# albertz/ParseOggVorbis

Measured on AMD Instinct MI355X. Metric: audio packets/sec (blocksize 2048, stereo), higher is better.
Workload: dtype f32; 1 GPU; config3: 65536 stereo packets, blocksize 2048, 64 streams x 1024, floor+coupling+IMDCT+window+overlap-add; packets_per_gpu=65536, parallelism=streams sharded over 1 GPU(s), no data-path collective

## Files before the change

parseoggvorbis_amd/csrc/vorbis_synth_hip.hip:

```cpp
#include <hip/hip_runtime.h>

#include <math.h>
#include <stdarg.h>
#include <stdio.h>
#include <string.h>

#include <algorithm>
#include <cmath>
#include <mutex>
#include <numeric>
#include <string>
#include <vector>

#include <stdlib.h>

#include "vsyn_device.h"
#include "vsyn_staged.h"
#include "vsyn_prep.h"
#include "vsyn_fused.h"
#include "vsyn_fused_u.h"
#include "vsyn_vq.h"
#include "vsyn_pcm.h"
#include "vsyn_features.h"
#include "vsyn_spectral.h"
// ... 486 lines not shown
        for (int i = 0; i + 1 < VQ_NSTAMPS; ++i) sum[i] += (double)host[u][i];
      }
      if (pk) {
        fprintf(stderr, "[vq stamps] %llu waves, %.1f packets each; s_memtime ticks per packet:", waves, (double)pk / waves);
        for (int i = 0; i + 1 < VQ_NSTAMPS; ++i) fprintf(stderr, " %d:%.0f", i, sum[i] / pk);
        fprintf(stderr, "\n");
      }
    }
  }
#endif
#ifdef PREP_STAMPS
  {
    static unsigned long long host[8192][PREP_NSTAMPS];
    if (hipMemcpyFromSymbol(host, HIP_SYMBOL(g_prep_stamps), sizeof(host)) == hipSuccess) {
      unsigned long long t_first = ~0ull;
      for (int u = 0; u < 8192; ++u)
        if (host[u][7] && host[u][5] < t_first) t_first = host[u][5];
      for (unsigned role = 0; role < 2; ++role) {
        double sum[5] = {0}, st = 0, en = 0, en_max = 0, st_max = 0;
        unsigned long long waves = 0;
        for (int u = 0; u < 8192; ++u) {
          if (host[u][7] != 1ull + role) continue;
          ++waves;
          for (int i = 0; i < 5; ++i) sum[i] += (double)host[u][i];
          const double a = (double)(host[u][5] - t_first) / 100.0, b = (double)(host[u][6] - t_first) / 100.0;
          st += a;
          en += b;
          if (a > st_max) st_max = a;
          if (b > en_max) en_max = b;
        }
        if (!waves) continue;
        static const char* nm[5] = {"header + stream state", "scan in front of the chunk", "descriptors, scan, PktInfo", "floor role: descriptors, floor ids", "floor role: chains"};
        fprintf(stderr, "prep stamps, %s role: %llu waves; start %.2f us (latest %.2f), end %.2f us (latest %.2f) after the launch's first wave\n",
                role ? "floor" : "layout", waves, st / waves, st_max, en / waves, en_max);
        for (int i = 0; i < 5; ++i)
          if (sum[i] > 0) fprintf(stderr, "  %-36s %8.0f cycles\n", nm[i], sum[i] / waves);
      }
    }
  }
#endif
#ifdef VSYN_STAMPS
  {
    static unsigned long long host[8192][VSYN_NSTAMPS];
    if (hipMemcpyFromSymbol(host, HIP_SYMBOL(g_vsyn_stamps), sizeof(host)) == hipSuccess) {
      double sum[VSYN_NSTAMPS] = {0};
      unsigned long long waves = 0, pk = 0;
      for (int u = 0; u < 8192; ++u) {
        if (!host[u][VSYN_NSTAMPS - 1]) continue;
        ++waves;
        pk += host[u][VSYN_NSTAMPS - 1];
        for (int i = 0; i + 1 < VSYN_NSTAMPS; ++i) sum[i] += (double)host[u][i];
      }
      if (pk) {
        static const char* nm[VSYN_NSTAMPS - 1] = {"loop", "residue+handoff+couple", "loads+floor setup", "floor product", "mirror+pre-rot", "partner wait 2",
                                                   "fft512", "post+window+overlap", "stores / short pass: stores", "short: descriptors", "short: rows", "short: couple+floor", "short: fft+window", "-", "-"};
        double tot = 0;
        for (int i = 0; i + 1 < VSYN_NSTAMPS; ++i) tot += sum[i];
        fprintf(stderr, "vsyn stamps: %llu waves, %llu wave-packets, %.0f cycles per wave-packet\n", waves, pk, tot / pk);
        for (int i = 0; i + 1 < VSYN_NSTAMPS; ++i) fprintf(stderr, "  %-26s %8.0f cycles  %5.1f %%\n", nm[i], sum[i] / pk, 100.0 * sum[i] / tot);
      }
    }
  }
#endif
  fused_tables_destroy(&h->fused);
  u_tables_destroy(&h->utab);
  if (h->side) (void)hipStreamDestroy(h->side);
  if (h->pre) (void)hipStreamDestroy(h->pre);
  if (h->host_stream) (void)hipStreamDestroy(h->host_stream);
  if (h->ev_join) (void)hipEventDestroy(h->ev_join);
  if (h->ev_self) (void)hipEventDestroy(h->ev_self);
  if (h->ev_reset) (void)hipEventDestroy(h->ev_reset);
  for (uint32_t b = 0; b < vsyn_handle::WS_RING; ++b)
    if (h->ev_pre_done[b]) (void)hipEventDestroy(h->ev_pre_done[b]);
  for (uint32_t b = 0; b < vsyn_handle::EV_RING; ++b)
    if (h->ev_ring[b]) (void)hipEventDestroy(h->ev_ring[b]);
  if (h->d_const) (void)hipFree(h->d_const);
  if (h->d_vq) (void)hipFree(h->d_vq);
  h->st_curve.release(); h->st_vqpk.release(); h->st_cls.release(); h->st_ent.release();
  if (h->d_state) (void)hipFree(h->d_state);
  if (h->d_carry) (void)hipFree(h->d_carry);
  if (h->d_status) (void)hipFree(h->d_status);
  h->ws_count.release();
  h->ws_chunks.release();
  for (uint32_t b = 0; b < vsyn_handle::WS_RING; ++b) {
    h->ws_list[b].release(); h->ws_info[b].release(); h->ws_seg[b].release(); h->ws_segmap[b].release(); h->ws_fy[b].release(); h->ws_runcls[b].release();
  }
  h->ws_env.release(); h->ws_blk.release();
  h->st_pk.release(); h->st_seg.release(); h->st_ys.release(); h->st_fy.release(); h->st_res.release(); h->st_pcm.release();
  h->st_env.release(); h->st_blk.release(); h->st_emit.release();
  h->st_sum.release(); h->st_conv.release(); h->st_frames.release();
  for (auto& ev : h->events) {
    (void)hipEventDestroy(ev.first);
    (void)hipEventDestroy(ev.second);
  }
  delete h;
}

uint32_t vsyn_ys_stride(const vsyn_handle* h) { return h ? h->H.ys_stride : 0; }
uint32_t vsyn_channels(const vsyn_handle* h) { return h ? h->H.channels : 0; }
uint32_t vsyn_fused_paths(const vsyn_handle* h) { return h ? (h->fused_mask | (h->vq_tables_in_lds ? 0x100u : 0u)) : 0; }
size_t vsyn_const_block_bytes(const vsyn_handle* h) { return h ? h->host_const.size() : 0; }

int vsyn_profile_enable(vsyn_handle* h, int on) {
  if (!h) return VSYN_ERR_INVALID;
  h->profile = on != 0;
  if (on >= 1 && on <= 3) h->profile_which = on;
  return VSYN_OK;
}

int vsyn_profile_read(vsyn_handle* h, double* mean_ms, uint32_t* launches, const char** kernel_name) {
  if (!h) return VSYN_ERR_INVALID;
  std::lock_guard<std::mutex> lk(h->mu);
// ... 1695 lines not shown
```

parseoggvorbis_amd/csrc/vsyn_fused.h:

```cpp
#pragma once
#include <hip/hip_runtime.h>

#include "vsyn_device.h"

#ifndef FUSED_WAVES
#define FUSED_WAVES 16
#endif
#ifndef FUSED_MIN_WAVES_PER_SIMD
#define FUSED_MIN_WAVES_PER_SIMD 4
#endif
#define FUSED_XSLOTS 576
#ifndef VSYN_KNOCKOUT
#define VSYN_KNOCKOUT 0
#endif
#ifdef VSYN_STAMPS
#define VSYN_NSTAMPS 16
__device__ unsigned long long g_vsyn_stamps[8192][VSYN_NSTAMPS];
#define STAMP(i)                                                  \
  do {                                                            \
    __builtin_amdgcn_sched_barrier(0);                            \
    const unsigned long long t_ = __builtin_readcyclecounter();   \
    st_acc[i] += t_ - st_last;                                    \
    st_last = t_;                                                 \
    __builtin_amdgcn_sched_barrier(0);                            \
  } while (0)
#else
#define STAMP(i) do { } while (0)
#endif

struct FusedLdsImage {
  float2 pre[8][64];
  float2 post[8][64];
  float2 tw1[8][64];
  float2 tw2[8][8];
  float win[2][2][8][64];
  float invdb[260];
  float2 pre_s[64];
  float2 post_s[64];
  float2 tws[6][64];
  float wsl[2][64];
  float2 post8[8][8];
  float wsl8[2][8][8];
};

struct FusedTables {
  uint8_t* d_binseg = nullptr;
  FusedLdsImage* d_lds = nullptr;
  int waves_per_cu = 12;
  int coupling_mode = 0;
};

struct FusedArgs {
  const uint8_t* cb;
  const uint8_t* binseg;
  const FusedLdsImage* lds_image;
  const vsyn_packet* packets;
  const vsyn_segment* segs;
  const PktInfo* info;
  const SegInfo* sinfo;
  uint16_t* curve;
  const uint8_t* run_cls;
  const float* residue;
  const uint16_t* fy;
  float* pcm;
  float* carry;
  DevStatus* status;
  uint64_t plane_stride;
  uint32_t S, R, fused_ok, coupling_mode, runs_per_seg;
};
// ... 73 lines not shown
  asm volatile("" ::: "memory");
  uint32_t spins = 0;
  while (!dead && *(const volatile lds_u32*)flag < v) {
    __builtin_amdgcn_s_sleep(2);
    if (++spins > (1u << 24)) {
      if ((threadIdx.x & 63u) == 0) atomicOr(&status->flags, VSYN_ST_BAD_SEGMENT);
      dead = true;
    }
  }
  asm volatile("" ::: "memory");
}

__device__ __forceinline__ float min0(float a) {
  float r;
  asm("v_min_f32 %0, 0, %1" : "=v"(r) : "v"(a));
  return r;
}
__device__ __forceinline__ float max0(float a) {
  float r;
  asm("v_max_f32 %0, 0, %1" : "=v"(r) : "v"(a));
  return r;
}
__device__ __forceinline__ float couple_mag(float m, float a) {
  const float na = min0(a);
  return m + (m > 0.f ? na : -na);
}
__device__ __forceinline__ float couple_ang(float m, float a) {
  const float pa = max0(a);
  return m + (m > 0.f ? -pa : pa);
}

typedef uint32_t u32x8 __attribute__((ext_vector_type(8)));
static_assert(sizeof(PktInfo) == 32, "PktInfo is fetched as one s_load_dwordx8");
struct PktScalars {
  uint64_t res_off;
  uint32_t out_pos, emit, used, own, widx, mapping, lng, bad;
};
__device__ __forceinline__ PktScalars pkt_fields(const u32x8 r) {
  PktScalars k;
  k.res_off = (uint64_t)r[0] | ((uint64_t)r[1] << 32);
  k.out_pos = r[2];
  k.emit = r[3];
  k.used = r[4];
  k.own = r[5];
  k.widx = r[6] >> 24;
  k.mapping = r[7] & 0xFFu;
  k.lng = (r[6] >> 16) & 0xFFu;
  k.bad = (r[7] >> 8) & 0xFFu;
  return k;
}
__device__ __forceinline__ PktScalars pkt_load(const PktInfo* p) {
  typedef const __attribute__((address_space(4))) u32x8* const_words;
  return pkt_fields(*(const_words)(uintptr_t)p);
}

enum { K_REG = 0, K_LDS = 1, K_CARRY = 2 };
__device__ __forceinline__ uint32_t bitrev6(uint32_t l) { return __brev(l) >> 26; }

template <int ROLE, bool TAPC>
__device__ __forceinline__ uint32_t fused_short_pass(const FusedArgs& A, const FusedLdsImage& T, float2* __restrict__ xb, const float2* __restrict__ pxb,
                                                     float2* seg2, lds_f32* cbuf, lds_u32* my_flags, const lds_u32* partner_flags, const uint32_t lane,
                                                     const vsyn_segment sg, const SegInfo si, const uint32_t q, const uint32_t qa, const uint32_t qb,
                                                     const uint32_t C, const uint32_t c, float* plane, const PktInfo* ip, const uint32_t epoch,
                                                     const uint32_t prev_kind, const uint32_t prev_half, float (&P)[8], const uint32_t bseg0,
                                                     const uint32_t sidx, const uint32_t xsl, const uint32_t posts, const uint32_t ys_stride, bool& hand_over_out
#ifdef VSYN_STAMPS
                                                     , unsigned long long (&st_acc)[VSYN_NSTAMPS], unsigned long long& st_last
#endif
                                                     ) {
  constexpr uint32_t MS = 128u, ML = 1024u;
  const ConstHeader* H = hdr_of(A.cb);
  typedef uint32_t u32x4 __attribute__((ext_vector_type(4)));
  const uint32_t idx = min(q + (lane & 7u), qb - 1u);
  const u32x4 da = ((const u32x4*)(ip + idx))[0], db = ((const u32x4*)(ip + idx))[1];
  const uint32_t map0 = __builtin_amdgcn_readfirstlane(db[3] & 0xFFu);
  const bool cand = lane < 8u && q + lane < qb;
  const uint64_t okm = __ballot(cand && !((db[3] >> 8) & 0xFFu) && !((db[2] >> 16) & 0xFFu) && (db[3] & 0xFFu) == map0);
  const uint32_t Jp = (uint32_t)__builtin_ctzll(~okm);
  STAMP(9);
  const uint32_t qn = q + Jp, p0 = sg.first_packet + q;
  const uint32_t emit_l = q + (lane & 7u) < qa ? 0u : da[3];
  float2 raw[8];
  uint32_t vrow[8];
#pragma unroll
  for (uint32_t t = 0; t < 8; ++t) {
    const uint32_t tc = min(t, Jp - 1u);
    const uint64_t off = ((uint64_t)__builtin_amdgcn_readlane(da[1], tc) << 32) | (uint32_t)__builtin_amdgcn_readlane(da[0], tc);
    raw[t] = (VSYN_KNOCKOUT & 256) ? f2(0.001f * (float)lane, 0.002f) : ((const float2*)(A.residue + off + (size_t)c * MS))[lane];
    vrow[t] = (A.fy + ((size_t)(p0 + tc) * C + c) * ys_stride)[sidx];
  }
#pragma unroll
  for (uint32_t t = 0; t < 8; ++t)
    if (t >= Jp) raw[t] = f2(0.f, 0.f);
  float2 r[8];
  if (ROLE != 0 && !(VSYN_KNOCKOUT & 512)) {
#pragma unroll
    for (int t = 0; t < 8; ++t) xb[t * 64 + lane] = raw[t];
    STAMP(10);
    pair_post(&my_flags[0], epoch);
    pair_wait(&partner_flags[0], epoch);
#pragma unroll
    for (int t = 0; t < 8; ++t) {
      const float2 oth = pxb[t * 64 + lane];
      r[t] = ROLE == 1 ? f2(couple_mag(raw[t].x, oth.x), couple_mag(raw[t].y, oth.y)) : f2(couple_ang(oth.x, raw[t].x), couple_ang(oth.y, raw[t].y));
    }
    pair_post(&my_flags[1], epoch);
// ... 163 lines not shown
          *(float2*)(up + 16 * j) = f2(oh_s[j], n_s[j]);
          *(float2*)(dn - 16 * j) = f2(n_m[j], oh_m[j]);
        }
      }
    } else if (emit) {
#pragma unroll
      for (int j = 0; j < 4; ++j) {
        const uint32_t s = 2u * kap + 16u * j;
        const uint32_t f0 = s + shift, f1 = s + 1u + shift, f2m = MS - 2u - s + shift, f3m = MS - 1u - s + shift;
        if (f0 < emit) out[f0] = oh_s[j];
        if (f1 < emit) out[f1] = n_s[j];
        if (f2m < emit) out[f2m] = n_m[j];
        if (f3m < emit) out[f3m] = oh_m[j];
      }
    }
  }
  (void)next_emit;
  (void)next_out;
  if ((last_of_segment || hand_over) && jo == Jp - 1u) {
    const size_t carry_half = (size_t)H->max_streams * C * ML;
    float* cout = A.carry + (si.parity_in ^ 1u) * carry_half + ((size_t)sg.stream * C + c) * ML;
#pragma unroll
    for (int k = 0; k < 8; ++k) {
      const uint32_t f = kap + 8u * k;
      const uint32_t s = k >= 4 ? 2u * f - 64u : 63u - 2u * f, sm = MS - 1u - s;
      const float v_s = Pn[k] * wl1[k], v_m = Pn[k] * wl0[k];
      if (last_of_segment) {
        cout[s] = v_s;
        cout[sm] = v_m;
      } else {
        cbuf[s] = v_s;
        cbuf[sm] = v_m;
      }
    }
  }
  {
    const int from = (int)((Jp - 1u) * 8u + kap);
#pragma unroll
    for (int k = 0; k < 8; ++k) P[k] = __shfl(Pn[k], from);
  }
  if (__any(floor_bad)) {
    if (floor_bad) raise_status(A.status, VSYN_ST_FLOOR_VALUE, floor_bad_pkt);
    vmem_drain();
  }
  hand_over_out = hand_over;
  return Jp;
}


template <int ROLE, bool MIXED, bool TAPC, bool RING = false>
__device__ __forceinline__ void fused_run(const FusedArgs& A, const FusedLdsImage& T, float2* __restrict__ xb, const float2* __restrict__ pxb, float4* __restrict__ seg,
                                          lds_f32* cbuf, lds_u32* my_flags, const lds_u32* partner_flags, const uint32_t lane0, const uint32_t g,
                                          const vsyn_segment sg, const SegInfo si, const uint32_t qa, const uint32_t qb, const uint32_t C, const uint32_t c,
                                          const RingLds& rl = RingLds()) {
  static_assert(!(RING && MIXED), "ring mode is a steady-run mode");
  constexpr uint32_t STEP = RING ? 8u : 1u;
  constexpr uint32_t ML = 1024;
  const uint8_t* __restrict__ cb = A.cb;
  const ConstHeader* H = hdr_of(cb);
  const uint32_t num = sg.num_packets;

  float P[8];
#pragma unroll
  for (int k = 0; k < 8; ++k) P[k] = 0.f;
  uint32_t prev_next_long = 1;
  uint32_t prev_kind = K_REG;
  uint32_t prev_half = 0;
  float* const plane = A.pcm + ((size_t)g * C + c) * A.plane_stride;
  const float* cin = nullptr;

  const uint32_t seg_base = (uint32_t)(uintptr_t)(lds_u32*)seg;
  uint32_t bseg[8];
#pragma unroll
  for (int t = 0; t < 8; ++t) bseg[t] = seg_base | (seg_base << 16);
  uint32_t sidx = 0, xsl = 0;
  int cur_floor = -1;
  uint32_t vrow = 0;
  bool vrow_ok = false;

  const uint32_t ys_stride = __builtin_amdgcn_readfirstlane(H->ys_stride);
  const MapConst* const maps = (const MapConst*)(cb + H->off_map);
  const FloorConst* const floors = (const FloorConst*)(cb + H->off_floor);
  uint32_t cur_map = 0xFFFFFFFFu, map_floor = 0, posts = 0;

  const uint32_t q0 = RING ? ((rl.slot == 7u && qa) ? qa - 1u : qa + rl.slot) : (qa ? qa - 1 : 0);
  if (RING && q0 >= qb) return;
  bool ring_dead = false;
  const PktInfo* const ip = A.info + __builtin_amdgcn_readfirstlane(sg.first_packet);
  PktScalars pi = pkt_load(ip + q0);
  float2 raw[8];
  bool raw_ahead = false;
  bool dma_ahead = false;
  uint32_t dma_younger = 0;
  auto issue_dma = [&](uint64_t off, const uint32_t ln) {
    const char* gsrc = (const char*)(A.residue + off) + 16u * ln;
#pragma unroll
    for (int i = 0; i < 4; ++i)
      __builtin_amdgcn_global_load_lds((const __attribute__((address_space(1))) void*)(gsrc + 1024 * i),
                                       (__attribute__((address_space(3))) void*)((lds_u32*)xb + 256 * i), 16, 0, 0);
  };
  if (!MIXED) {
    const float2* src = (const float2*)(A.residue + pi.res_off + (size_t)c * ML) + lane0;
#pragma unroll
    for (int t = 0; t < 8; ++t) raw[t] = stream_load2(src + 64 * t);
  }
  if (MIXED && qa == 0 && si.has_carry && !pi.bad) {
    const size_t carry_half = (size_t)H->max_streams * C * ML;
    cin = A.carry + si.parity_in * carry_half + ((size_t)sg.stream * C + c) * ML;
    const bool carry_long = si.carry_n == 2u * ML;
    prev_half = si.carry_n / 2u;
    if (carry_long && pi.lng) {
      prev_kind = K_CARRY;
    } else {
      const uint32_t base = carry_long ? 448u : 0u;
      if (carry_long)
        for (uint32_t i = lane0; i < min(448u, pi.emit); i += 64) plane[pi.out_pos + i] = cin[i];
      cbuf[lane0] = cin[base + lane0];
      cbuf[lane0 + 64u] = cin[base + lane0 + 64u];
      prev_kind = K_LDS;
    }
  }
  uint32_t lane_v = lane0;
  vmem_drain();
#ifdef VSYN_STAMPS
  unsigned long long st_acc[VSYN_NSTAMPS] = {0, 0, 0, 0, 0, 0, 0, 0, 0, 0, 0, 0, 0, 0, 0, 0};
  unsigned long long st_last = __builtin_readcyclecounter();
#endif
  uint32_t q = q0;
  for (uint32_t it = 0; q < qb; ++it, q += STEP) {
    STAMP(0);
    asm volatile("" : "+v"(lane_v));
    const uint32_t lane = lane_v;
    const uint32_t kappa = ((lane & 7u) << 3) | (lane >> 3);
    const uint32_t p = sg.first_packet + q;
    const bool halo = q < qa, has_next = q + STEP < qb;
    const PktScalars pin = pkt_load(ip + (has_next ? q + STEP : q));
    if (RING) prev_next_long = q ? (pkt_load(ip + q - 1u).widx >> 1) & 1u : 1u;
    const bool lng = !MIXED || pi.lng != 0u;
    const bool nlng = !MIXED || pin.lng != 0u;
    const uint32_t M = lng ? ML : 128u;
    if (MIXED && pi.bad) {
#pragma unroll
      for (int k = 0; k < 8; ++k) P[k] = 0.f;
      prev_kind = K_REG;
      prev_half = 0;
      vrow_ok = false;
      pi = pin;
      continue;
    }
    if (pi.mapping != cur_map) {
      cur_map = pi.mapping;
      {
        typedef const __attribute__((address_space(4))) uint32_t* kptr;
        const uint32_t w = *(kptr)(uintptr_t)((const uint8_t*)maps[cur_map].chfloor + (c & ~3u));
        map_floor = (w >> (8u * (c & 3u))) & 0xFFu;
      }
    }
    if (MIXED && !lng) {
      if (cur_floor != (int)map_floor) {
        const FloorConst* fc = floors + map_floor;
        posts = __builtin_amdgcn_readfirstlane(fc->posts);
        const uint8_t* bs = A.binseg + (size_t)map_floor * ML;
        const uint32_t seg_base0 = (uint32_t)(uintptr_t)(lds_u32*)seg;
#pragma unroll
        for (int t = 0; t < 8; ++t) {
          const uint32_t two = *(const uint16_t*)(bs + 2u * (lane + 64u * t));
          bseg[t] = (seg_base0 + 8u * (two & 0xFFu)) | ((seg_base0 + 8u * (two >> 8)) << 16);
        }
        const bool in = lane < posts;
        sidx = in ? fc->sorted_idx[lane] : 0u;
        xsl = in ? fc->xs_sorted[lane] : 0u;
        cur_floor = (int)map_floor;
        vmem_drain();
      }
      bool ho = false;
      const uint32_t Jp = fused_short_pass<ROLE, TAPC>(A, T, xb, pxb, (float2*)seg, cbuf, my_flags, partner_flags, lane, sg, si, q, qa, qb, C, c, plane, ip, it + 1u,
                                                 prev_kind, prev_half, P, bseg[0], sidx, xsl, posts, ys_stride, ho
#ifdef VSYN_STAMPS
                                                 , st_acc, st_last
#endif
                                                 );
      prev_kind = ho ? K_LDS : K_REG;
      prev_half = 128u;
// ... 133 lines not shown
          typedef float lds_vf2 __attribute__((ext_vector_type(2)));
          const lds_vf2 ev = *(const __attribute__((address_space(3))) lds_vf2*)(uintptr_t)addr;
          sgm[i] = f2(ev.x, ev.y);
        }
#pragma unroll
        for (int i = 0; i < 4; ++i) {
          const int b = 4 * grp + i;
          const uint32_t ix = (uint32_t)__builtin_fmaf(xf0 + (float)(128 * (b >> 1) + (b & 1)), sgm[i].x, sgm[i].y);
          fl[b] = T.invdb[ix];
          if (TAPC) ci[b] = ix;
        }
      }
      if (TAPC && ((pi.own >> c) & 1u)) {
        uint32_t* dst = (uint32_t*)(A.curve + pi.res_off + (size_t)c * (L ? ML : 128u)) + lane;
#pragma unroll
        for (int t = 0; t < 8; ++t)
          if (t == 0 || L) dst[64 * t] = ci[2 * t] | (ci[2 * t + 1] << 16);
      }
#pragma unroll
      for (int t = 0; t < 8; ++t)
        if (t == 0 || L) r[t] = f2(r[t].x * fl[2 * t], r[t].y * fl[2 * t + 1]);
    };

    const uint32_t emit = halo ? 0u : pi.emit;
    float* out = plane + pi.out_pos;
    const uint32_t cur_next_long = (pi.widx >> 1) & 1u;
    const bool last_of_segment = q == num - 1;
    const bool hand_over = MIXED && has_next && !pin.bad && (nlng != lng);
    if (lng) {
      if (!(VSYN_KNOCKOUT & 2)) floor_product(true);
      STAMP(3);
      float2 z[8];
#pragma unroll
      for (int t = 0; t < 8; ++t) {
        const float im = __shfl(r[7 - t].y, 63 - (int)lane);
        z[t] = cmulf(f2(r[t].x, im), T.pre[t][lane]);
      }
      STAMP(4);
      if (ROLE != 0 && !(VSYN_KNOCKOUT & 1)) pair_wait(&partner_flags[1], it + 1);
      STAMP(5);
      if (!(VSYN_KNOCKOUT & 4)) fft512_wave(z, xb, &T, lane);
      STAMP(6);
      if (MIXED) {
        dma_ahead = has_next && nlng && !pin.bad;
        dma_younger = 0xFFu;
        if (dma_ahead) {
          asm volatile("s_waitcnt lgkmcnt(0)" ::: "memory");
          issue_dma(pin.res_off + (uint64_t)c * ML, lane);
          dma_younger = 0;
        }
      }
#pragma unroll
      for (int k = 0; k < 8; ++k) z[k] = cmulf(z[k], T.post[k][lane]);
      if (RING) {
        const uint32_t tag = q + 2u - qa;
        if (q != q0) ring_wait(&rl.succ_flags[1], tag - 8u, A.status, ring_dead);
#pragma unroll
        for (int k = 0; k < 8; ++k) rl.mine[64 * k + lane] = k >= 4 ? z[k].y : -z[k].x;
        pair_post(&rl.flags[0], tag);
        if (!halo && q != 0u) {
          ring_wait(&rl.pred_flags[0], tag - 1u, A.status, ring_dead);
#pragma unroll
          for (int k = 0; k < 8; ++k) P[k] = rl.pred[64 * k + lane];
          pair_post(&rl.flags[1], tag - 1u);
        } else {
#pragma unroll
          for (int k = 0; k < 8; ++k) P[k] = 0.f;
        }
      }

      const float (*TL)[8][64] = T.win[pi.widx & 1u];
      const float (*TR)[8][64] = T.win[prev_next_long];
      const uint32_t shift = (!MIXED || prev_half != 128u) ? 0u : 0u - 448u;
      const bool fast_store = emit == ML && (!MIXED || shift == 0u) && (((uintptr_t)out & 7u) == 0);
      float oh_s[4], oh_m[4], n_s[4], n_m[4];
      float wl0[8], wl1[8], wr0[8], wr1[8];
#pragma unroll
      for (int k = 0; k < 8; ++k) {
        wl0[k] = TL[0][k][lane];
        wl1[k] = TL[1][k][lane];
      }
      if (MIXED && prev_kind != K_REG) {
#pragma unroll
        for (int k = 0; k < 8; ++k) {
          P[k] = 1.f;
          wr0[k] = 0.f;
          wr1[k] = 0.f;
        }
        if (prev_kind == K_LDS) {
          const bool up = kappa >= 32u;
          const float c0 = cbuf[up ? 2u * kappa - 64u : 63u - 2u * kappa];
          const float c1 = cbuf[up ? 191u - 2u * kappa : 64u + 2u * kappa];
          wr1[7] = up ? c0 : 0.f;
          wr0[7] = up ? c1 : 0.f;
          wr1[0] = up ? 0.f : c0;
          wr0[0] = up ? 0.f : c1;
        } else {
#pragma unroll
          for (int k = 0; k < 8; ++k) {
            const uint32_t m = kappa + 64u * k;
            const uint32_t sk = k >= 4 ? 2u * m - 512u : 511u - 2u * m;
            wr1[k] = cin[sk];
            wr0[k] = cin[1023u - sk];
          }
        }
      } else if (TR == TL) {
#pragma unroll
        for (int k = 0; k < 8; ++k) {
          wr0[k] = wl0[k];
          wr1[k] = wl1[k];
        }
      } else {
#pragma unroll
        for (int k = 0; k < 8; ++k) {
          wr0[k] = TR[0][k][lane];
          wr1[k] = TR[1][k][lane];
        }
      }
#pragma unroll
      for (int j = 0; j < 4; ++j) {
        const int kh = 4 + j, kl = 3 - j;
        const float cch = z[kh].x, ccl = -z[kl].y;
        const float ah_s = P[kh] * wr1[kh], ah_m = P[kh] * wr0[kh], al_s = P[kl] * wr1[kl], al_m = P[kl] * wr0[kl];
        oh_s[j] = ah_s + cch * wl0[kh];
        oh_m[j] = ah_m + (-cch) * wl1[kh];
        const float ol_s = al_s + ccl * wl0[kl];
        const float ol_m = al_m + (-ccl) * wl1[kl];
        P[kh] = z[kh].y;
        P[kl] = -z[kl].x;
        n_s[j] = __shfl(ol_s, 63 - (int)lane);
        n_m[j] = __shfl(ol_m, 63 - (int)lane);
      }
      if (!MIXED) vmem_drain();
      STAMP(7);
      if (VSYN_KNOCKOUT & 8) {
        float acc = 0.f;
#pragma unroll
        for (int j = 0; j < 4; ++j) acc += oh_s[j] + n_s[j] + n_m[j] + oh_m[j];
        if (acc == 12345.678f) out[lane] = acc;
      } else if (fast_store) {
        if (MIXED && dma_younger == 0u) dma_younger = 8u;
        float* up = out + 2u * kappa;
        float* dn = out + 1022u - 2u * kappa;
#pragma unroll
        for (int j = 0; j < 4; ++j) {
          if (!MIXED) {
            stream_store2(up + 128 * j, oh_s[j], n_s[j]);
            stream_store2(dn - 128 * j, n_m[j], oh_m[j]);
          } else {
            *(float2*)(up + 128 * j) = f2(oh_s[j], n_s[j]);
            *(float2*)(dn - 128 * j) = f2(n_m[j], oh_m[j]);
          }
        }
      } else if (emit) {
        if (MIXED) dma_younger = 0xFFu;
#pragma unroll
        for (int j = 0; j < 4; ++j) {
          const uint32_t s = 2u * kappa + 128u * j;
          const uint32_t f0 = s + shift, f1 = s + 1u + shift, f2m = 1022u - s + shift, f3m = 1023u - s + shift;
          if (f0 < emit) out[f0] = oh_s[j];
          if (f1 < emit) out[f1] = n_s[j];
          if (f2m < emit) out[f2m] = n_m[j];
          if (f3m < emit) out[f3m] = oh_m[j];
        }
      }
      STAMP(8);
      if (MIXED && (last_of_segment || hand_over)) dma_younger = 0xFFu;
      if (last_of_segment || hand_over) {
        const size_t carry_half = (size_t)H->max_streams * C * ML;
        float* cout = A.carry + (si.parity_in ^ 1u) * carry_half + ((size_t)sg.stream * C + c) * ML;
        float* nxt = plane + pin.out_pos;
        const float (*TN)[8][64] = T.win[cur_next_long];
#pragma unroll
        for (int k = 0; k < 8; ++k) {
          const uint32_t m = kappa + 64u * k;
          const uint32_t s = k >= 4 ? 2u * m - 512u : 511u - 2u * m;
          const float v_s = P[k] * TN[1][k][lane], v_m = P[k] * TN[0][k][lane];
          if (last_of_segment) {
            cout[s] = v_s;
            cout[1023u - s] = v_m;
          } else {
            const uint32_t sm = 1023u - s;
            if (s < 448u) {
              if (s < pin.emit) nxt[s] = v_s;
            } else if (s < 576u) {
              cbuf[s - 448u] = v_s;
            }
            if (sm < 448u) {
              if (sm < pin.emit) nxt[sm] = v_m;
            } else if (sm < 576u) {
              cbuf[sm - 448u] = v_m;
            }
          }
        }
        if (!MIXED) vmem_drain();
      }
    } else {
    }
    if (MIXED) {
      prev_kind = hand_over ? K_LDS : K_REG;
      prev_half = M;
    }
    if (__any(floor_bad)) {
      if (lane == 0) raise_status(A.status, VSYN_ST_FLOOR_VALUE, p);
      vmem_drain();
    }
    prev_next_long = cur_next_long;
    pi = pin;
  }
#ifdef VSYN_STAMPS
  if (lane0 == 0) {
    const uint32_t unit = blockIdx.x * FUSED_WAVES + (threadIdx.x >> 6);
    if (unit < 8192)
      for (int i = 0; i < VSYN_NSTAMPS; ++i) g_vsyn_stamps[unit][i] = i == VSYN_NSTAMPS - 1 ? (unsigned long long)(qb - q0) : st_acc[i];
  }
#endif
}

static_assert(FUSED_WAVES % 2 == 0, "the two channel waves of a run must share a workgroup");
template <bool TAPC>
__device__ __forceinline__ void fused_kernel_body(const FusedArgs& A) {
  struct Lds {
    float4 seg[FUSED_WAVES][64];
    uint32_t flag[FUSED_WAVES][4];
    FusedLdsImage t;
    float2 x[FUSED_WAVES][FUSED_XSLOTS];
    float ring[FUSED_WAVES][8 * 64];
  };
  __shared__ Lds s_lds;
  FusedLdsImage& s_t = s_lds.t;
  float2 (&s_x)[FUSED_WAVES][FUSED_XSLOTS] = s_lds.x;
  float4 (&s_seg)[FUSED_WAVES][64] = s_lds.seg;
  uint32_t (&s_flag)[FUSED_WAVES][4] = s_lds.flag;
  static_assert(sizeof(s_lds.seg) + sizeof(s_lds.flag) < 65536, "floor entry addresses are packed into 16 bits");
  const ConstHeader* H = hdr_of(A.cb);
  const uint32_t wave = __builtin_amdgcn_readfirstlane(threadIdx.x >> 6);
  const uint32_t lane = threadIdx.x & 63u;
  const uint32_t C = H->channels;
  const uint32_t per_seg = A.runs_per_seg * C;
  const uint32_t unit = blockIdx.x * FUSED_WAVES + wave;
  const uint32_t g = __builtin_amdgcn_readfirstlane(unit / per_seg);
  const uint32_t rem = unit - g * per_seg;
  const uint32_t run = __builtin_amdgcn_readfirstlane(rem / C), c = __builtin_amdgcn_readfirstlane(rem % C);
  vsyn_segment sg = {};
  SegInfo si = {};
  uint32_t cls = 0xFFu;
  bool seg_ok = false;
  if (g < A.S) {
    sg = A.segs[g];
    if (sg.stream < H->max_streams && !(sg.residue_off & 3)) {
      seg_ok = true;
      si = A.sinfo[g];
      cls = __builtin_amdgcn_readfirstlane((uint32_t)A.run_cls[(size_t)g * A.runs_per_seg + run]);
    }
  }
  const uint32_t qa = run * A.R;
  const uint32_t qb = min(sg.num_packets, qa + A.R);
  const bool active = (cls == 1u && (A.fused_ok & 1u)) || (cls == 2u && (A.fused_ok & 2u));
  if (!__syncthreads_or(active ? 1 : 0)) return;
  {
    const uint4* src = (const uint4*)A.lds_image;
    uint4* dst = (uint4*)&s_t;
    for (uint32_t i = threadIdx.x; i < sizeof(FusedLdsImage) / 16; i += FUSED_WAVES * 64) dst[i] = src[i];
    if (threadIdx.x < FUSED_WAVES * 4) (&s_flag[0][0])[threadIdx.x] = 0u;
  }
  static_assert(FUSED_WAVES == 16, "ring mode: 8 slots x 2 channels");
  const uint32_t unit0 = blockIdx.x * FUSED_WAVES;
  const bool one_seg = unit0 / per_seg == (unit0 + FUSED_WAVES - 1u) / per_seg;
  const bool ring_ok = C == 2u && one_seg && g < A.S && (A.fused_ok & 1u) && seg_ok && (cls == 1u || qa >= sg.num_packets);
  const bool ring = __syncthreads_and(ring_ok ? 1 : 0);
  if (!ring && !active) return;
  const uint32_t mag = A.coupling_mode == 1 ? 0u : 1u;
  const int role = (A.coupling_mode == 0 || C < 2) ? 0 : (c == mag ? 1 : 2);
  const uint32_t pw = role ? (wave ^ 1u) : wave;
  lds_u32* mf = (lds_u32*)s_flag[wave];
  const lds_u32* pf = (const lds_u32*)s_flag[pw];
  lds_f32* cbw = (lds_f32*)((float*)s_seg[wave] + 128);
  if (ring) {
    const uint32_t slot = wave >> 1, pred = ((slot + 7u) & 7u) * 2u + c, succ = ((slot + 1u) & 7u) * 2u + c;
    RingLds rl;
    rl.mine = (lds_f32*)s_lds.ring[wave];
    rl.pred = (const lds_f32*)s_lds.ring[pred];
    rl.flags = (lds_u32*)&s_flag[wave][2];
    rl.pred_flags = (const lds_u32*)&s_flag[pred][2];
    rl.succ_flags = (const lds_u32*)&s_flag[succ][2];
    rl.slot = slot;
    const uint32_t ca = qa - slot * A.R, ce = min(sg.num_packets, ca + 8u * A.R);
    if (role == 0) fused_run<0, false, TAPC, true>(A, s_t, s_x[wave], s_x[pw], s_seg[wave], cbw, mf, pf, lane, g, sg, si, ca, ce, C, c, rl);
    else if (role == 1) fused_run<1, false, TAPC, true>(A, s_t, s_x[wave], s_x[pw], s_seg[wave], cbw, mf, pf, lane, g, sg, si, ca, ce, C, c, rl);
    else fused_run<2, false, TAPC, true>(A, s_t, s_x[wave], s_x[pw], s_seg[wave], cbw, mf, pf, lane, g, sg, si, ca, ce, C, c, rl);
  } else if (cls == 1u) {
    if (role == 0) fused_run<0, false, TAPC>(A, s_t, s_x[wave], s_x[pw], s_seg[wave], cbw, mf, pf, lane, g, sg, si, qa, qb, C, c);
    else if (role == 1) fused_run<1, false, TAPC>(A, s_t, s_x[wave], s_x[pw], s_seg[wave], cbw, mf, pf, lane, g, sg, si, qa, qb, C, c);
    else fused_run<2, false, TAPC>(A, s_t, s_x[wave], s_x[pw], s_seg[wave], cbw, mf, pf, lane, g, sg, si, qa, qb, C, c);
  } else {
    if (role == 0) fused_run<0, true, TAPC>(A, s_t, s_x[wave], s_x[pw], s_seg[wave], cbw, mf, pf, lane, g, sg, si, qa, qb, C, c);
    else if (role == 1) fused_run<1, true, TAPC>(A, s_t, s_x[wave], s_x[pw], s_seg[wave], cbw, mf, pf, lane, g, sg, si, qa, qb, C, c);
    else fused_run<2, true, TAPC>(A, s_t, s_x[wave], s_x[pw], s_seg[wave], cbw, mf, pf, lane, g, sg, si, qa, qb, C, c);
  }
}

__global__ void __launch_bounds__(FUSED_WAVES * 64, FUSED_MIN_WAVES_PER_SIMD) vsyn_fused_kernel(const FusedArgs A) { fused_kernel_body<false>(A); }
__global__ void __launch_bounds__(FUSED_WAVES * 64, FUSED_MIN_WAVES_PER_SIMD) vsyn_fused_tap_kernel(const FusedArgs A) { fused_kernel_body<true>(A); }

static inline bool fused_supported(const ConstHeader& H) {
  return H.bs[1] == 2048 && H.bs[0] <= 2048 && H.channels <= 2;
}

static inline int fused_coupling_mode(const ConstHeader& H, const uint8_t* host_const) {
  const MapConst* mp = (const MapConst*)(host_const + H.off_map);
  int mode = -2;
  for (uint32_t k = 0; k < H.num_modes; ++k) {
    if (!H.mode_blockflag[k]) continue;
    const MapConst& m = mp[H.mode_mapping[k]];
    if (m.ncoup > 1) return -1;
    const int cur = m.ncoup == 0 ? 0 : (m.coup[0] == 0 ? 1 : 2);
    if (mode == -2) mode = cur;
    else if (mode != cur) return -1;
  }
  return mode == -2 ? 0 : mode;
}

static inline uint32_t fused_ok_mask(const ConstHeader& H, const uint8_t* host_const);

static inline bool fused_setup_ok(const ConstHeader& H, const uint8_t* host_const) {
  if (!fused_supported(H)) return false;
  const FloorConst* fl = (const FloorConst*)(host_const + H.off_floor);
  for (uint32_t f = 0; f < H.num_floors; ++f)
    if (fl[f].posts > 64) return false;
  return fused_coupling_mode(H, host_const) >= 0;
}

static inline uint32_t fused_ok_mask(const ConstHeader& H, const uint8_t* host_const) {
  if (!fused_setup_ok(H, host_const)) return 0;
  uint32_t mask = 1;
  if (H.bs[0] == 256) {
    const MapConst* mp = (const MapConst*)(host_const + H.off_map);
    const int want = fused_coupling_mode(H, host_const);
    bool same = true;
    for (uint32_t k = 0; k < H.num_modes; ++k) {
      const MapConst& m = mp[H.mode_mapping[k]];
      const int cur = m.ncoup == 0 ? 0 : (m.ncoup == 1 ? (m.coup[0] == 0 ? 1 : 2) : -1);
      same = same && cur == want;
    }
    if (same) mask |= 2;
  }
  return mask;
}

static inline hipError_t fused_tables_create(const ConstHeader& H, const uint8_t* host_const, FusedTables* ft, bool debug) {
  const uint32_t half = H.bs[1] / 2;
// ... 187 lines not shown
```

Before: 271.5 million packets/s.

## Prefetch first packet rows during kernel prologue and defer ring consume

Starts the first packet's residue rows DMA into LDS and the LDS image loads before the block-wide barrier. Segment headers are read as scalar words, and one LDS vote replaces two syncthreads reductions. In ring mode, the predecessor overlap wait is deferred until after the current-window products are computed, and the wave's own tail is reloaded from its ring slot. This aims to hide prologue latency and inter-wave ring waits. It adds LDS for votes, extra register pressure, and more complex control flow. Extended stamp instrumentation is also added.

```diff
diff --git a/parseoggvorbis_amd/csrc/vorbis_synth_hip.hip b/parseoggvorbis_amd/csrc/vorbis_synth_hip.hip
--- a/parseoggvorbis_amd/csrc/vorbis_synth_hip.hip
+++ b/parseoggvorbis_amd/csrc/vorbis_synth_hip.hip
@@ -562,12 +562,31 @@
         for (int i = 0; i + 1 < VSYN_NSTAMPS; ++i) sum[i] += (double)host[u][i];
       }
       if (pk) {
+        constexpr int PER_PACKET = 15;
         static const char* nm[VSYN_NSTAMPS - 1] = {"loop", "residue+handoff+couple", "loads+floor setup", "floor product", "mirror+pre-rot", "partner wait 2",
-                                                   "fft512", "post+window+overlap", "stores / short pass: stores", "short: descriptors", "short: rows", "short: couple+floor", "short: fft+window", "-", "-"};
+                                                   "fft512", "post+window+overlap", "stores / short pass: stores", "short: descriptors", "short: rows", "short: couple+floor", "short: fft+window",
+                                                   "ring wait: successor read", "ring wait: predecessor post", "head: start -> 1st rows", "tail: last stores -> end", "whole wave", "-"};
         double tot = 0;
-        for (int i = 0; i + 1 < VSYN_NSTAMPS; ++i) tot += sum[i];
+        for (int i = 0; i < PER_PACKET; ++i) tot += sum[i];
         fprintf(stderr, "vsyn stamps: %llu waves, %llu wave-packets, %.0f cycles per wave-packet\n", waves, pk, tot / pk);
-        for (int i = 0; i + 1 < VSYN_NSTAMPS; ++i) fprintf(stderr, "  %-26s %8.0f cycles  %5.1f %%\n", nm[i], sum[i] / pk, 100.0 * sum[i] / tot);
+        for (int i = 0; i < PER_PACKET; ++i) fprintf(stderr, "  %-26s %8.0f cycles  %5.1f %%\n", nm[i], sum[i] / pk, 100.0 * sum[i] / tot);
+        for (int i = PER_PACKET; i < 18; ++i) fprintf(stderr, "  %-26s %8.0f cycles per wave  %5.1f %% of the wave\n", nm[i], sum[i] / waves, 100.0 * sum[i] / sum[17]);
+        double ssum[8][4] = {{0}};
+        unsigned long long sw[8] = {0}, sp[8] = {0};
+        for (int u = 0; u < 8192; ++u) {
+          if (!host[u][VSYN_NSTAMPS - 1] || !host[u][18]) continue;
+          const int sl = (int)host[u][18] - 1;
+          ++sw[sl];
+          sp[sl] += host[u][VSYN_NSTAMPS - 1];
+          ssum[sl][0] += (double)host[u][13];
+          ssum[sl][1] += (double)host[u][14];
+          ssum[sl][2] += (double)host[u][15];
+          ssum[sl][3] += (double)host[u][17];
+        }
+        for (int sl = 0; sl < 8; ++sl)
+          if (sw[sl])
+            fprintf(stderr, "  ring slot %d: %llu waves, %.1f packets each; per packet wait successor %.0f, wait predecessor %.0f; per wave head %.0f, whole %.0f cycles\n", sl,
+                    sw[sl], (double)sp[sl] / sw[sl], ssum[sl][0] / sp[sl], ssum[sl][1] / sp[sl], ssum[sl][2] / sw[sl], ssum[sl][3] / sw[sl]);
       }
     }
   }
diff --git a/parseoggvorbis_amd/csrc/vsyn_fused.h b/parseoggvorbis_amd/csrc/vsyn_fused.h
--- a/parseoggvorbis_amd/csrc/vsyn_fused.h
+++ b/parseoggvorbis_amd/csrc/vsyn_fused.h
@@ -13,8 +13,14 @@
 #ifndef VSYN_KNOCKOUT
 #define VSYN_KNOCKOUT 0
 #endif
+#ifndef VSYN_RING_LATE
+#define VSYN_RING_LATE 1
+#endif
+#ifndef VSYN_EARLY_HEAD
+#define VSYN_EARLY_HEAD 1
+#endif
 #ifdef VSYN_STAMPS
-#define VSYN_NSTAMPS 16
+#define VSYN_NSTAMPS 20
 __device__ unsigned long long g_vsyn_stamps[8192][VSYN_NSTAMPS];
 #define STAMP(i)                                                  \
   do {                                                            \
@@ -194,6 +200,22 @@
 __device__ __forceinline__ PktScalars pkt_load(const PktInfo* p) {
   typedef const __attribute__((address_space(4))) u32x8* const_words;
   return pkt_fields(*(const_words)(uintptr_t)p);
+}
+
+#define FUSED_NO_EARLY 0xFFFFFFFFu
+struct EarlyHead {
+  uint32_t q0 = FUSED_NO_EARLY;
+  PktScalars pi = {};
+#ifdef VSYN_STAMPS
+  unsigned long long t0 = 0, head = 0;
+#endif
+};
+__device__ __forceinline__ void rows_to_image(const float* rows, float2* xb, const uint32_t lane) {
+  const char* gsrc = (const char*)rows + 16u * lane;
+#pragma unroll
+  for (int i = 0; i < 4; ++i)
+    __builtin_amdgcn_global_load_lds((const __attribute__((address_space(1))) void*)(gsrc + 1024 * i),
+                                     (__attribute__((address_space(3))) void*)((lds_u32*)xb + 256 * i), 16, 0, 0);
 }
 
 enum { K_REG = 0, K_LDS = 1, K_CARRY = 2 };
@@ -463,7 +485,7 @@
 __device__ __forceinline__ void fused_run(const FusedArgs& A, const FusedLdsImage& T, float2* __restrict__ xb, const float2* __restrict__ pxb, float4* __restrict__ seg,
                                           lds_f32* cbuf, lds_u32* my_flags, const lds_u32* partner_flags, const uint32_t lane0, const uint32_t g,
                                           const vsyn_segment sg, const SegInfo si, const uint32_t qa, const uint32_t qb, const uint32_t C, const uint32_t c,
-                                          const RingLds& rl = RingLds()) {
+                                          const RingLds& rl = RingLds(), const EarlyHead& eh = EarlyHead()) {
   static_assert(!(RING && MIXED), "ring mode is a steady-run mode");
   constexpr uint32_t STEP = RING ? 8u : 1u;
   constexpr uint32_t ML = 1024;
@@ -498,7 +520,8 @@
   if (RING && q0 >= qb) return;
   bool ring_dead = false;
   const PktInfo* const ip = A.info + __builtin_amdgcn_readfirstlane(sg.first_packet);
-  PktScalars pi = pkt_load(ip + q0);
+  const bool early = !MIXED && eh.q0 == q0;
+  PktScalars pi = early ? eh.pi : pkt_load(ip + q0);
   float2 raw[8];
   bool raw_ahead = false;
   bool dma_ahead = false;
@@ -511,10 +534,21 @@
                                        (__attribute__((address_space(3))) void*)((lds_u32*)xb + 256 * i), 16, 0, 0);
   };
   if (!MIXED) {
-    const float2* src = (const float2*)(A.residue + pi.res_off + (size_t)c * ML) + lane0;
-#pragma unroll
-    for (int t = 0; t < 8; ++t) raw[t] = stream_load2(src + 64 * t);
-  }
+    if (early) {
+      vmem_drain();
+#pragma unroll
+      for (int t = 0; t < 8; ++t) raw[t] = xb[t * 64 + lane0];
+    } else {
+      const float2* src = (const float2*)(A.residue + pi.res_off + (size_t)c * ML) + lane0;
+#pragma unroll
+      for (int t = 0; t < 8; ++t) raw[t] = stream_load2(src + 64 * t);
+    }
+  }
+#ifdef VSYN_STAMPS
+  __builtin_amdgcn_sched_barrier(0);
+  const unsigned long long st_head = early ? eh.head : __builtin_readcyclecounter() - eh.t0;
+  __builtin_amdgcn_sched_barrier(0);
+#endif
   if (MIXED && qa == 0 && si.has_carry && !pi.bad) {
     const size_t carry_half = (size_t)H->max_streams * C * ML;
     cin = A.carry + si.parity_in * carry_half + ((size_t)sg.stream * C + c) * ML;
@@ -534,12 +568,20 @@
   uint32_t lane_v = lane0;
   vmem_drain();
 #ifdef VSYN_STAMPS
-  unsigned long long st_acc[VSYN_NSTAMPS] = {0, 0, 0, 0, 0, 0, 0, 0, 0, 0, 0, 0, 0, 0, 0, 0};
+  unsigned long long st_acc[VSYN_NSTAMPS] = {0, 0, 0, 0, 0, 0, 0, 0, 0, 0, 0, 0, 0, 0, 0, 0, 0, 0, 0, 0};
+  unsigned long long st_iters = 0;
   unsigned long long st_last = __builtin_readcyclecounter();
+#endif
+#ifdef VSYN_RING_STAGGER
+  if (RING)
+    for (uint32_t i = 0; i < rl.slot; ++i) __builtin_amdgcn_s_sleep(VSYN_RING_STAGGER);
 #endif
   uint32_t q = q0;
   for (uint32_t it = 0; q < qb; ++it, q += STEP) {
     STAMP(0);
+#ifdef VSYN_STAMPS
+    ++st_iters;
+#endif
     asm volatile("" : "+v"(lane_v));
     const uint32_t lane = lane_v;
     const uint32_t kappa = ((lane & 7u) << 3) | (lane >> 3);
@@ -779,14 +821,12 @@
       }
 #pragma unroll
       for (int k = 0; k < 8; ++k) z[k] = cmulf(z[k], T.post[k][lane]);
-      if (RING) {
+      auto ring_consume = [&]() {
         const uint32_t tag = q + 2u - qa;
-        if (q != q0) ring_wait(&rl.succ_flags[1], tag - 8u, A.status, ring_dead);
-#pragma unroll
-        for (int k = 0; k < 8; ++k) rl.mine[64 * k + lane] = k >= 4 ? z[k].y : -z[k].x;
-        pair_post(&rl.flags[0], tag);
-        if (!halo && q != 0u) {
+        if (!halo && q != 0u && !(VSYN_KNOCKOUT & 1024)) {
+          STAMP(7);
           ring_wait(&rl.pred_flags[0], tag - 1u, A.status, ring_dead);
+          STAMP(14);
 #pragma unroll
           for (int k = 0; k < 8; ++k) P[k] = rl.pred[64 * k + lane];
           pair_post(&rl.flags[1], tag - 1u);
@@ -794,6 +834,18 @@
 #pragma unroll
           for (int k = 0; k < 8; ++k) P[k] = 0.f;
         }
+      };
+      if (RING) {
+        const uint32_t tag = q + 2u - qa;
+        if (!(VSYN_KNOCKOUT & 1024)) {
+          STAMP(7);
+          if (q != q0) ring_wait(&rl.succ_flags[1], tag - 8u, A.status, ring_dead);
+          STAMP(13);
+#pragma unroll
+          for (int k = 0; k < 8; ++k) rl.mine[64 * k + lane] = k >= 4 ? z[k].y : -z[k].x;
+          pair_post(&rl.flags[0], tag);
+        }
+        if (!VSYN_RING_LATE) ring_consume();
       }
 
       const float (*TL)[8][64] = T.win[pi.widx & 1u];
@@ -844,17 +896,33 @@
           wr1[k] = TR[1][k][lane];
         }
       }
+      float bh_s[4], bh_m[4], bl_s[4], bl_m[4];
 #pragma unroll
       for (int j = 0; j < 4; ++j) {
         const int kh = 4 + j, kl = 3 - j;
         const float cch = z[kh].x, ccl = -z[kl].y;
+        bh_s[j] = cch * wl0[kh];
+        bh_m[j] = (-cch) * wl1[kh];
+        bl_s[j] = ccl * wl0[kl];
+        bl_m[j] = (-ccl) * wl1[kl];
+      }
+      if (RING && VSYN_RING_LATE) {
+#pragma unroll
+        for (int j = 0; j < 4; ++j) asm volatile("" : "+v"(bh_s[j]), "+v"(bh_m[j]), "+v"(bl_s[j]), "+v"(bl_m[j]));
+        ring_consume();
+      }
+#pragma unroll
+      for (int j = 0; j < 4; ++j) {
+        const int kh = 4 + j, kl = 3 - j;
         const float ah_s = P[kh] * wr1[kh], ah_m = P[kh] * wr0[kh], al_s = P[kl] * wr1[kl], al_m = P[kl] * wr0[kl];
-        oh_s[j] = ah_s + cch * wl0[kh];
-        oh_m[j] = ah_m + (-cch) * wl1[kh];
-        const float ol_s = al_s + ccl * wl0[kl];
-        const float ol_m = al_m + (-ccl) * wl1[kl];
-        P[kh] = z[kh].y;
-        P[kl] = -z[kl].x;
+        oh_s[j] = ah_s + bh_s[j];
+        oh_m[j] = ah_m + bh_m[j];
+        const float ol_s = al_s + bl_s[j];
+        const float ol_m = al_m + bl_m[j];
+        if (!RING) {
+          P[kh] = z[kh].y;
+          P[kl] = -z[kl].x;
+        }
         n_s[j] = __shfl(ol_s, 63 - (int)lane);
         n_m[j] = __shfl(ol_m, 63 - (int)lane);
       }
@@ -898,6 +966,10 @@
         float* cout = A.carry + (si.parity_in ^ 1u) * carry_half + ((size_t)sg.stream * C + c) * ML;
         float* nxt = plane + pin.out_pos;
         const float (*TN)[8][64] = T.win[cur_next_long];
+        if (RING) {
+#pragma unroll
+          for (int k = 0; k < 8; ++k) P[k] = (VSYN_KNOCKOUT & 1024) ? 0.f : rl.mine[64 * k + lane];
+        }
 #pragma unroll
         for (int k = 0; k < 8; ++k) {
           const uint32_t m = kappa + 64u * k;
@@ -936,10 +1008,19 @@
     pi = pin;
   }
 #ifdef VSYN_STAMPS
+  {
+    __builtin_amdgcn_sched_barrier(0);
+    const unsigned long long t_end = __builtin_readcyclecounter();
+    st_acc[15] = st_head;
+    st_acc[16] = t_end - st_last;
+    st_acc[17] = t_end - eh.t0;
+    st_acc[18] = RING ? rl.slot + 1u : 0u;
+    st_acc[VSYN_NSTAMPS - 1] = st_iters;
+  }
   if (lane0 == 0) {
     const uint32_t unit = blockIdx.x * FUSED_WAVES + (threadIdx.x >> 6);
     if (unit < 8192)
-      for (int i = 0; i < VSYN_NSTAMPS; ++i) g_vsyn_stamps[unit][i] = i == VSYN_NSTAMPS - 1 ? (unsigned long long)(qb - q0) : st_acc[i];
+      for (int i = 0; i < VSYN_NSTAMPS; ++i) g_vsyn_stamps[unit][i] = st_acc[i];
   }
 #endif
 }
@@ -950,6 +1031,7 @@
   struct Lds {
     float4 seg[FUSED_WAVES][64];
     uint32_t flag[FUSED_WAVES][4];
+    uint32_t vote[FUSED_WAVES];
     FusedLdsImage t;
     float2 x[FUSED_WAVES][FUSED_XSLOTS];
     float ring[FUSED_WAVES][8 * 64];
@@ -963,6 +1045,16 @@
   const ConstHeader* H = hdr_of(A.cb);
   const uint32_t wave = __builtin_amdgcn_readfirstlane(threadIdx.x >> 6);
   const uint32_t lane = threadIdx.x & 63u;
+  EarlyHead eh;
+#ifdef VSYN_STAMPS
+  eh.t0 = __builtin_readcyclecounter();
+#endif
+#if VSYN_EARLY_HEAD
+  constexpr uint32_t IMG_VECS = sizeof(FusedLdsImage) / 16, WG = FUSED_WAVES * 64;
+  static_assert(sizeof(FusedLdsImage) % 16 == 0 && IMG_VECS > WG && IMG_VECS <= 2 * WG, "the image is staged as two 16-byte pieces per thread");
+  const uint4 img0 = ((const uint4*)A.lds_image)[threadIdx.x];
+  const uint4 img1 = ((const uint4*)A.lds_image)[min(threadIdx.x + WG, IMG_VECS - 1u)];
+#endif
   const uint32_t C = H->channels;
   const uint32_t per_seg = A.runs_per_seg * C;
   const uint32_t unit = blockIdx.x * FUSED_WAVES + wave;
@@ -973,6 +1065,29 @@
   SegInfo si = {};
   uint32_t cls = 0xFFu;
   bool seg_ok = false;
+#if VSYN_EARLY_HEAD
+  if (g < A.S) {
+    typedef const __attribute__((address_space(4))) uint32_t* kwords;
+    static_assert(sizeof(vsyn_segment) == 24 && sizeof(SegInfo) == 16, "read as 6 and 4 words");
+    const kwords ws = (kwords)(uintptr_t)(A.segs + g), wi = (kwords)(uintptr_t)(A.sinfo + g);
+    const size_t ci = (size_t)g * A.runs_per_seg + run;
+    const uint32_t cw = *(kwords)((uintptr_t)(A.run_cls + ci) & ~(uintptr_t)3);
+    sg.stream = ws[0];
+    sg.first_packet = ws[1];
+    sg.num_packets = ws[2];
+    sg.flags = ws[3];
+    sg.residue_off = (uint64_t)ws[4] | ((uint64_t)ws[5] << 32);
+    const uint32_t i0 = wi[0], i1 = wi[1], i2 = wi[2], i3 = wi[3];
+    if (sg.stream < H->max_streams && !(sg.residue_off & 3)) {
+      seg_ok = true;
+      si.has_carry = i0;
+      si.carry_n = i1;
+      si.parity_in = i2;
+      si.total_emit = i3;
+      cls = (cw >> (8u * (uint32_t)((uintptr_t)(A.run_cls + ci) & 3u))) & 0xFFu;
+    }
+  }
+#else
   if (g < A.S) {
     sg = A.segs[g];
     if (sg.stream < H->max_streams && !(sg.residue_off & 3)) {
@@ -981,9 +1096,43 @@
       cls = __builtin_amdgcn_readfirstlane((uint32_t)A.run_cls[(size_t)g * A.runs_per_seg + run]);
     }
   }
+#endif
   const uint32_t qa = run * A.R;
   const uint32_t qb = min(sg.num_packets, qa + A.R);
   const bool active = (cls == 1u && (A.fused_ok & 1u)) || (cls == 2u && (A.fused_ok & 2u));
+  static_assert(FUSED_WAVES == 16, "ring mode: 8 slots x 2 channels");
+  const uint32_t unit0 = blockIdx.x * FUSED_WAVES;
+  const bool one_seg = unit0 / per_seg == (unit0 + FUSED_WAVES - 1u) / per_seg;
+  const bool ring_ok = C == 2u && one_seg && g < A.S && (A.fused_ok & 1u) && seg_ok && (cls == 1u || qa >= sg.num_packets);
+#if VSYN_EARLY_HEAD
+  {
+    const uint32_t slot = wave >> 1, ca = qa - slot * A.R;
+    uint32_t q0 = FUSED_NO_EARLY;
+    if (ring_ok) q0 = (slot == 7u && ca) ? ca - 1u : ca + slot;
+    else if (seg_ok && cls == 1u && (A.fused_ok & 1u) && qa < sg.num_packets) q0 = qa ? qa - 1u : 0u;
+    if (q0 < sg.num_packets) {
+      eh.pi = pkt_load(A.info + sg.first_packet + q0);
+      if (eh.pi.lng && !eh.pi.bad) {
+        eh.q0 = q0;
+        rows_to_image(A.residue + eh.pi.res_off + (size_t)c * 1024u, s_x[wave], lane);
+#ifdef VSYN_STAMPS
+        eh.head = __builtin_readcyclecounter() - eh.t0;
+#endif
+      }
+    }
+  }
+  {
+    uint4* dst = (uint4*)&s_t;
+    dst[threadIdx.x] = img0;
+    if (threadIdx.x + WG < IMG_VECS) dst[threadIdx.x + WG] = img1;
+    if (threadIdx.x < FUSED_WAVES * 4) (&s_flag[0][0])[threadIdx.x] = 0u;
+    if (lane == 0) s_lds.vote[wave] = (active ? 1u : 0u) | (ring_ok ? 2u : 0u);
+  }
+  lds_barrier();
+  const uint32_t votes = s_lds.vote[lane & (FUSED_WAVES - 1u)];
+  if (!__any(votes & 1u)) return;
+  const bool ring = __all((votes & 2u) != 0u);
+#else
   if (!__syncthreads_or(active ? 1 : 0)) return;
   {
     const uint4* src = (const uint4*)A.lds_image;
@@ -991,11 +1140,8 @@
     for (uint32_t i = threadIdx.x; i < sizeof(FusedLdsImage) / 16; i += FUSED_WAVES * 64) dst[i] = src[i];
     if (threadIdx.x < FUSED_WAVES * 4) (&s_flag[0][0])[threadIdx.x] = 0u;
   }
-  static_assert(FUSED_WAVES == 16, "ring mode: 8 slots x 2 channels");
-  const uint32_t unit0 = blockIdx.x * FUSED_WAVES;
-  const bool one_seg = unit0 / per_seg == (unit0 + FUSED_WAVES - 1u) / per_seg;
-  const bool ring_ok = C == 2u && one_seg && g < A.S && (A.fused_ok & 1u) && seg_ok && (cls == 1u || qa >= sg.num_packets);
   const bool ring = __syncthreads_and(ring_ok ? 1 : 0);
+#endif
   if (!ring && !active) return;
   const uint32_t mag = A.coupling_mode == 1 ? 0u : 1u;
   const int role = (A.coupling_mode == 0 || C < 2) ? 0 : (c == mag ? 1 : 2);
@@ -1013,17 +1159,17 @@
     rl.succ_flags = (const lds_u32*)&s_flag[succ][2];
     rl.slot = slot;
     const uint32_t ca = qa - slot * A.R, ce = min(sg.num_packets, ca + 8u * A.R);
-    if (role == 0) fused_run<0, false, TAPC, true>(A, s_t, s_x[wave], s_x[pw], s_seg[wave], cbw, mf, pf, lane, g, sg, si, ca, ce, C, c, rl);
-    else if (role == 1) fused_run<1, false, TAPC, true>(A, s_t, s_x[wave], s_x[pw], s_seg[wave], cbw, mf, pf, lane, g, sg, si, ca, ce, C, c, rl);
-    else fused_run<2, false, TAPC, true>(A, s_t, s_x[wave], s_x[pw], s_seg[wave], cbw, mf, pf, lane, g, sg, si, ca, ce, C, c, rl);
+    if (role == 0) fused_run<0, false, TAPC, true>(A, s_t, s_x[wave], s_x[pw], s_seg[wave], cbw, mf, pf, lane, g, sg, si, ca, ce, C, c, rl, eh);
+    else if (role == 1) fused_run<1, false, TAPC, true>(A, s_t, s_x[wave], s_x[pw], s_seg[wave], cbw, mf, pf, lane, g, sg, si, ca, ce, C, c, rl, eh);
+    else fused_run<2, false, TAPC, true>(A, s_t, s_x[wave], s_x[pw], s_seg[wave], cbw, mf, pf, lane, g, sg, si, ca, ce, C, c, rl, eh);
   } else if (cls == 1u) {
-    if (role == 0) fused_run<0, false, TAPC>(A, s_t, s_x[wave], s_x[pw], s_seg[wave], cbw, mf, pf, lane, g, sg, si, qa, qb, C, c);
-    else if (role == 1) fused_run<1, false, TAPC>(A, s_t, s_x[wave], s_x[pw], s_seg[wave], cbw, mf, pf, lane, g, sg, si, qa, qb, C, c);
-    else fused_run<2, false, TAPC>(A, s_t, s_x[wave], s_x[pw], s_seg[wave], cbw, mf, pf, lane, g, sg, si, qa, qb, C, c);
+    if (role == 0) fused_run<0, false, TAPC>(A, s_t, s_x[wave], s_x[pw], s_seg[wave], cbw, mf, pf, lane, g, sg, si, qa, qb, C, c, RingLds(), eh);
+    else if (role == 1) fused_run<1, false, TAPC>(A, s_t, s_x[wave], s_x[pw], s_seg[wave], cbw, mf, pf, lane, g, sg, si, qa, qb, C, c, RingLds(), eh);
+    else fused_run<2, false, TAPC>(A, s_t, s_x[wave], s_x[pw], s_seg[wave], cbw, mf, pf, lane, g, sg, si, qa, qb, C, c, RingLds(), eh);
   } else {
-    if (role == 0) fused_run<0, true, TAPC>(A, s_t, s_x[wave], s_x[pw], s_seg[wave], cbw, mf, pf, lane, g, sg, si, qa, qb, C, c);
-    else if (role == 1) fused_run<1, true, TAPC>(A, s_t, s_x[wave], s_x[pw], s_seg[wave], cbw, mf, pf, lane, g, sg, si, qa, qb, C, c);
-    else fused_run<2, true, TAPC>(A, s_t, s_x[wave], s_x[pw], s_seg[wave], cbw, mf, pf, lane, g, sg, si, qa, qb, C, c);
+    if (role == 0) fused_run<0, true, TAPC>(A, s_t, s_x[wave], s_x[pw], s_seg[wave], cbw, mf, pf, lane, g, sg, si, qa, qb, C, c, RingLds(), eh);
+    else if (role == 1) fused_run<1, true, TAPC>(A, s_t, s_x[wave], s_x[pw], s_seg[wave], cbw, mf, pf, lane, g, sg, si, qa, qb, C, c, RingLds(), eh);
+    else fused_run<2, true, TAPC>(A, s_t, s_x[wave], s_x[pw], s_seg[wave], cbw, mf, pf, lane, g, sg, si, qa, qb, C, c, RingLds(), eh);
   }
 }
 
```

Result: no change. 271.4 million packets/s (-0.0%).
